# VincentStimper/normalizing-flows

Hardware: NVIDIA H100
Metric: samples/sec forward_kld, 32-layer RQ-NSF d=64 batch=65536 (higher is better)
Workload: dtype f32

## Files before the change

normalizing-flows_b200/csrc/nfb_common.cuh:

```cuda
#pragma once
#include <cuda_runtime.h>
#include <cuda_bf16.h>
#include <cuda_fp16.h>
#include <stdint.h>
#include <stdio.h>

#define NFB_OK 0
#define NFB_ERR_CUDA 1
#define NFB_ERR_ARG 2
#define NFB_ERR_UNSUPPORTED 3
#define NFB_ERR_STATE 4

void nfb_set_error(const char* fmt, ...);

#define NFB_CUDA(call)                                                                   \
    do {                                                                                 \
        cudaError_t e__ = (call);                                                        \
        if (e__ != cudaSuccess) {                                                        \
            nfb_set_error("%s:%d: %s -> %s", __FILE__, __LINE__, #call,                  \
                          cudaGetErrorString(e__));                                      \
            return NFB_ERR_CUDA;                                                         \
        }                                                                                \
    } while (0)

// ... 51 lines not shown
        "selp.u32 %0, 1, 0, p;\n\t}"
        : "=r"(ok)
        : "r"(bar), "r"(parity)
        : "memory");
    return ok != 0;
}
static __device__ __noinline__ void fail_timeout(int* err, int tag) {
    if (err) atomicExch(err, tag);
    __threadfence_system();
    asm volatile("trap;");
}

__device__ __forceinline__ void mbar_wait(uint32_t bar, uint32_t parity, int* err, int tag) {
    if (mbar_try_wait(bar, parity)) return;
    long long t0 = clock64();
    while (!mbar_try_wait(bar, parity)) {
        if (clock64() - t0 > 4000000000LL) fail_timeout(err, tag);
    }
}

__device__ __forceinline__ void mbar_wait_warp(uint32_t bar, uint32_t parity, int* err, int tag) {
    if ((threadIdx.x & 31) == 0 && !mbar_try_wait(bar, parity)) {
        long long t0 = clock64();
        while (!mbar_try_wait(bar, parity)) {
            if (clock64() - t0 > 4000000000LL) fail_timeout(err, tag);
        }
    }
    __syncwarp();
}

__device__ __forceinline__ void bulk_g2s(uint32_t dst_smem, const void* src, uint32_t bytes,
                                         uint32_t bar) {
    asm volatile(
        "cp.async.bulk.shared::cluster.global.mbarrier::complete_tx::bytes [%0], [%1], %2, [%3];"
        ::"r"(dst_smem), "l"(src), "r"(bytes), "r"(bar)
        : "memory");
}
__device__ __forceinline__ void fence_proxy_async_smem() {
    asm volatile("fence.proxy.async.shared::cta;" ::: "memory");
}

__device__ __forceinline__ uint64_t wgmma_desc(uint32_t smem_addr, uint32_t lbo16 = 1, uint32_t sbo16 = 64) {
    return (uint64_t)((smem_addr & 0x3FFFFu) >> 4) | ((uint64_t)lbo16 << 16) | ((uint64_t)sbo16 << 32) | (1ull << 62);
}
__device__ __forceinline__ void wgmma_fence() { asm volatile("wgmma.fence.sync.aligned;" ::: "memory"); }
__device__ __forceinline__ void wgmma_commit() { asm volatile("wgmma.commit_group.sync.aligned;" ::: "memory"); }
template <int N> __device__ __forceinline__ void wgmma_wait() {
    asm volatile("wgmma.wait_group.sync.aligned %0;" ::"n"(N) : "memory");
}
template <int R> __device__ __forceinline__ void wgmma_hold(float (&d)[R]) {
#pragma unroll
    for (int i = 0; i < R; ++i) asm volatile("" : "+f"(d[i])::"memory");
}
__device__ __forceinline__ void wgmma_f16_n64(float (&d)[32], uint64_t a, uint64_t b, uint32_t scale_d) {
    asm volatile(
        "{\n\t.reg .pred p;\n\tsetp.ne.b32 p, %34, 0;\n\t"
        "wgmma.mma_async.sync.aligned.m64n64k16.f32.f16.f16 "
        "{"
        "%0,%1,%2,%3,%4,%5,%6,%7,%8,%9,%10,%11,%12,%13,%14,%15,"
        "%16,%17,%18,%19,%20,%21,%22,%23,%24,%25,%26,%27,%28,%29,%30,%31"
        "}, %32, %33, p, 1, 1, 0, 0;\n\t}"
        : "+f"(d[0]), "+f"(d[1]), "+f"(d[2]), "+f"(d[3]), "+f"(d[4]), "+f"(d[5]), "+f"(d[6]), "+f"(d[7]), "+f"(d[8]),
          "+f"(d[9]), "+f"(d[10]), "+f"(d[11]), "+f"(d[12]), "+f"(d[13]), "+f"(d[14]), "+f"(d[15]), "+f"(d[16]),
          "+f"(d[17]), "+f"(d[18]), "+f"(d[19]), "+f"(d[20]), "+f"(d[21]), "+f"(d[22]), "+f"(d[23]), "+f"(d[24]),
          "+f"(d[25]), "+f"(d[26]), "+f"(d[27]), "+f"(d[28]), "+f"(d[29]), "+f"(d[30]), "+f"(d[31])
        : "l"(a), "l"(b), "r"(scale_d));
}
__device__ __forceinline__ void wgmma_f16_n96(float (&d)[48], uint64_t a, uint64_t b, uint32_t scale_d) {
    asm volatile(
        "{\n\t.reg .pred p;\n\tsetp.ne.b32 p, %50, 0;\n\t"
        "wgmma.mma_async.sync.aligned.m64n96k16.f32.f16.f16 "
        "{"
        "%0,%1,%2,%3,%4,%5,%6,%7,%8,%9,%10,%11,%12,%13,%14,%15,"
        "%16,%17,%18,%19,%20,%21,%22,%23,%24,%25,%26,%27,%28,%29,%30,%31,"
        "%32,%33,%34,%35,%36,%37,%38,%39,%40,%41,%42,%43,%44,%45,%46,%47"
        "}, %48, %49, p, 1, 1, 0, 0;\n\t}"
        : "+f"(d[0]), "+f"(d[1]), "+f"(d[2]), "+f"(d[3]), "+f"(d[4]), "+f"(d[5]), "+f"(d[6]), "+f"(d[7]), "+f"(d[8]),
          "+f"(d[9]), "+f"(d[10]), "+f"(d[11]), "+f"(d[12]), "+f"(d[13]), "+f"(d[14]), "+f"(d[15]), "+f"(d[16]),
          "+f"(d[17]), "+f"(d[18]), "+f"(d[19]), "+f"(d[20]), "+f"(d[21]), "+f"(d[22]), "+f"(d[23]), "+f"(d[24]),
          "+f"(d[25]), "+f"(d[26]), "+f"(d[27]), "+f"(d[28]), "+f"(d[29]), "+f"(d[30]), "+f"(d[31]), "+f"(d[32]),
          "+f"(d[33]), "+f"(d[34]), "+f"(d[35]), "+f"(d[36]), "+f"(d[37]), "+f"(d[38]), "+f"(d[39]), "+f"(d[40]),
          "+f"(d[41]), "+f"(d[42]), "+f"(d[43]), "+f"(d[44]), "+f"(d[45]), "+f"(d[46]), "+f"(d[47])
        : "l"(a), "l"(b), "r"(scale_d));
}
__device__ __forceinline__ void wgmma_f16_n96_zero(float (&d)[48], uint64_t a, uint64_t b) {
    asm volatile(
        "wgmma.mma_async.sync.aligned.m64n96k16.f32.f16.f16 "
        "{"
        "%0,%1,%2,%3,%4,%5,%6,%7,%8,%9,%10,%11,%12,%13,%14,%15,"
        "%16,%17,%18,%19,%20,%21,%22,%23,%24,%25,%26,%27,%28,%29,%30,%31,"
        "%32,%33,%34,%35,%36,%37,%38,%39,%40,%41,%42,%43,%44,%45,%46,%47"
        "}, %48, %49, 0, 1, 1, 0, 0;"
        : "=f"(d[0]), "=f"(d[1]), "=f"(d[2]), "=f"(d[3]), "=f"(d[4]), "=f"(d[5]), "=f"(d[6]), "=f"(d[7]), "=f"(d[8]),
          "=f"(d[9]), "=f"(d[10]), "=f"(d[11]), "=f"(d[12]), "=f"(d[13]), "=f"(d[14]), "=f"(d[15]), "=f"(d[16]),
          "=f"(d[17]), "=f"(d[18]), "=f"(d[19]), "=f"(d[20]), "=f"(d[21]), "=f"(d[22]), "=f"(d[23]), "=f"(d[24]),
          "=f"(d[25]), "=f"(d[26]), "=f"(d[27]), "=f"(d[28]), "=f"(d[29]), "=f"(d[30]), "=f"(d[31]), "=f"(d[32]),
          "=f"(d[33]), "=f"(d[34]), "=f"(d[35]), "=f"(d[36]), "=f"(d[37]), "=f"(d[38]), "=f"(d[39]), "=f"(d[40]),
          "=f"(d[41]), "=f"(d[42]), "=f"(d[43]), "=f"(d[44]), "=f"(d[45]), "=f"(d[46]), "=f"(d[47])
        : "l"(a), "l"(b));
}
template <int TA = 0, int TB = 0>
__device__ __forceinline__ void wgmma_bf16_n64(float (&d)[32], uint64_t a, uint64_t b, uint32_t scale_d, uint32_t on = 1) {
    asm volatile(
        "{\n\t.reg .pred p, q;\n\tsetp.ne.b32 p, %34, 0;\n\tsetp.ne.b32 q, %37, 0;\n\t"
        "@q wgmma.mma_async.sync.aligned.m64n64k16.f32.bf16.bf16 "
        "{"
        "%0,%1,%2,%3,%4,%5,%6,%7,%8,%9,%10,%11,%12,%13,%14,%15,"
        "%16,%17,%18,%19,%20,%21,%22,%23,%24,%25,%26,%27,%28,%29,%30,%31"
        "}, %32, %33, p, 1, 1, %35, %36;\n\t}"
        : "+f"(d[0]), "+f"(d[1]), "+f"(d[2]), "+f"(d[3]), "+f"(d[4]), "+f"(d[5]), "+f"(d[6]), "+f"(d[7]), "+f"(d[8]),
          "+f"(d[9]), "+f"(d[10]), "+f"(d[11]), "+f"(d[12]), "+f"(d[13]), "+f"(d[14]), "+f"(d[15]), "+f"(d[16]),
          "+f"(d[17]), "+f"(d[18]), "+f"(d[19]), "+f"(d[20]), "+f"(d[21]), "+f"(d[22]), "+f"(d[23]), "+f"(d[24]),
          "+f"(d[25]), "+f"(d[26]), "+f"(d[27]), "+f"(d[28]), "+f"(d[29]), "+f"(d[30]), "+f"(d[31])
        : "l"(a), "l"(b), "r"(scale_d), "n"(TA), "n"(TB), "r"(on));
}
template <int TA = 0, int TB = 0>
__device__ __forceinline__ void wgmma_bf16_n128(float (&d)[64], uint64_t a, uint64_t b, uint32_t scale_d, uint32_t on = 1) {
    asm volatile(
        "{\n\t.reg .pred p, q;\n\tsetp.ne.b32 p, %66, 0;\n\tsetp.ne.b32 q, %69, 0;\n\t"
        "@q wgmma.mma_async.sync.aligned.m64n128k16.f32.bf16.bf16 "
        "{"
        "%0,%1,%2,%3,%4,%5,%6,%7,%8,%9,%10,%11,%12,%13,%14,%15,"
        "%16,%17,%18,%19,%20,%21,%22,%23,%24,%25,%26,%27,%28,%29,%30,%31,"
        "%32,%33,%34,%35,%36,%37,%38,%39,%40,%41,%42,%43,%44,%45,%46,%47,"
        "%48,%49,%50,%51,%52,%53,%54,%55,%56,%57,%58,%59,%60,%61,%62,%63"
        "}, %64, %65, p, 1, 1, %67, %68;\n\t}"
        : "+f"(d[0]), "+f"(d[1]), "+f"(d[2]), "+f"(d[3]), "+f"(d[4]), "+f"(d[5]), "+f"(d[6]), "+f"(d[7]), "+f"(d[8]),
          "+f"(d[9]), "+f"(d[10]), "+f"(d[11]), "+f"(d[12]), "+f"(d[13]), "+f"(d[14]), "+f"(d[15]), "+f"(d[16]),
          "+f"(d[17]), "+f"(d[18]), "+f"(d[19]), "+f"(d[20]), "+f"(d[21]), "+f"(d[22]), "+f"(d[23]), "+f"(d[24]),
          "+f"(d[25]), "+f"(d[26]), "+f"(d[27]), "+f"(d[28]), "+f"(d[29]), "+f"(d[30]), "+f"(d[31]), "+f"(d[32]),
          "+f"(d[33]), "+f"(d[34]), "+f"(d[35]), "+f"(d[36]), "+f"(d[37]), "+f"(d[38]), "+f"(d[39]), "+f"(d[40]),
          "+f"(d[41]), "+f"(d[42]), "+f"(d[43]), "+f"(d[44]), "+f"(d[45]), "+f"(d[46]), "+f"(d[47]), "+f"(d[48]),
          "+f"(d[49]), "+f"(d[50]), "+f"(d[51]), "+f"(d[52]), "+f"(d[53]), "+f"(d[54]), "+f"(d[55]), "+f"(d[56]),
          "+f"(d[57]), "+f"(d[58]), "+f"(d[59]), "+f"(d[60]), "+f"(d[61]), "+f"(d[62]), "+f"(d[63])
        : "l"(a), "l"(b), "r"(scale_d), "n"(TA), "n"(TB), "r"(on));
}

template <int N> __device__ __forceinline__ void setmaxnreg_dec() {
    asm volatile("setmaxnreg.dec.sync.aligned.u32 %0;" ::"n"(N));
}
template <int N> __device__ __forceinline__ void setmaxnreg_inc() {
    asm volatile("setmaxnreg.inc.sync.aligned.u32 %0;" ::"n"(N));
}

__device__ __forceinline__ uint32_t pack_bf16x2(float lo_elem, float hi_elem) {
    uint32_t r;
    asm("cvt.rn.bf16x2.f32 %0, %1, %2;" : "=r"(r) : "f"(hi_elem), "f"(lo_elem));
    return r;
}
__device__ __forceinline__ uint32_t pack_f16x2(float lo_elem, float hi_elem) {
    uint32_t r;
    asm("cvt.rn.f16x2.f32 %0, %1, %2;" : "=r"(r) : "f"(hi_elem), "f"(lo_elem));
    return r;
}
__device__ __forceinline__ float2 unpack_f16x2(uint32_t h) {
    return __half22float2(*reinterpret_cast<const __half2*>(&h));
}

__device__ __forceinline__ float warp_sum(float v) {
#pragma unroll
    for (int o = 16; o > 0; o >>= 1) v += __shfl_xor_sync(0xffffffffu, v, o);
    return v;
}

}
```

normalizing-flows_b200/csrc/nfb_fused_rqs.cu:

```cuda
#include <type_traits>

#include "nfb_kernels.h"
#include "nfb_spline.cuh"

namespace nfb {

constexpr int kRows = kFusedTileRows;
constexpr int kCons = 256;
constexpr int kFusedThreads = kCons + 128;
constexpr int kProducerRegs = 24, kConsumerRegs = 240;
constexpr uint32_t kTileA = 8192;
constexpr uint32_t kSlotBytes = 32768;
constexpr uint32_t kSlots = 3;
constexpr uint32_t kOffW = 8 * kTileA;
constexpr uint32_t kOffX = kOffW + kSlots * kSlotBytes;
constexpr int kStgLd = 52;
constexpr uint32_t kStgBytes = kRows * kStgLd * 4;
constexpr uint32_t kOffStg = kOffX + kRows * 64 * 4;
constexpr uint32_t kOffMisc = kOffStg + 2 * kStgBytes;
constexpr uint32_t kOffBars = kOffMisc + 4 * kRows * 4;
constexpr uint32_t kNumBars = 10;
constexpr uint32_t kOffUnitQ = kOffBars + kNumBars * 8;
constexpr uint32_t kFusedSmem = kOffUnitQ + 32;
static_assert(kFusedSmem <= 232448, "shared memory budget");
static_assert(2 * kFusedFeaturesPerChunk * 24 * 64 * 4 <= (int)kSlotBytes, "final-layer record must fit a ring slot");

constexpr int kBarWFull = 0 , kBarWEmpty = 3 , kBarUnit = 6 ;

__device__ __forceinline__ uint32_t xs_index(int r, int c) { return r * 64 + (c ^ (r & 31)); }

__device__ __forceinline__ uint32_t a_chunk_off(int r, int c8) {
    return (r >> 3) * 1024 + (r & 7) * 128 + ((c8 ^ (r & 7)) << 4);
}

__device__ __forceinline__ void st_shared_v4(uint32_t addr, uint32_t a, uint32_t b, uint32_t c,
                                             uint32_t d) {
    asm volatile("st.shared.v4.b32 [%0], {%1,%2,%3,%4};" ::"r"(addr), "r"(a), "r"(b), "r"(c), "r"(d)
                 : "memory");
}
__device__ __forceinline__ void st_shared_b32(uint32_t addr, uint32_t v) {
    asm volatile("st.shared.b32 [%0], %1;" ::"r"(addr), "r"(v) : "memory");
}
__device__ __forceinline__ void cons_bar_sync() {
    asm volatile("bar.sync 1, %0;" ::"n"(kCons) : "memory");
}
constexpr int kBarStgFull = 2, kBarStgFree = 3;
template <int ID> __device__ __forceinline__ void stg_bar_arrive() {
    __threadfence_block();
    asm volatile("bar.arrive %0, %1;" ::"n"(ID), "n"(kCons) : "memory");
}
template <int ID> __device__ __forceinline__ void stg_bar_wait() {
    asm volatile("bar.sync %0, %1;" ::"n"(ID), "n"(kCons) : "memory");
}
__device__ __forceinline__ void mbar_arrive_if(uint32_t bar, bool pred) {
    asm volatile("{\n\t.reg .pred p;\n\tsetp.ne.b32 p, %1, 0;\n\t@p mbarrier.arrive.shared::cta.b64 _, [%0];\n\t}"
                 ::"r"(bar), "r"((uint32_t)pred) : "memory");
}

__device__ __forceinline__ void split_store8(const float* v, uint32_t t0, uint32_t t1, uint32_t off) {
    uint32_t h[4], l[4];
#pragma unroll
    for (int i = 0; i < 4; ++i) {
        const float a = v[2 * i], b = v[2 * i + 1];
        h[i] = pack_f16x2(a, b);
        const float2 hf = unpack_f16x2(h[i]);
        l[i] = pack_f16x2(a - hf.x, b - hf.y);
    }
    st_shared_v4(t0 + off, h[0], h[1], h[2], h[3]);
    st_shared_v4(t1 + off, l[0], l[1], l[2], l[3]);
}
template <typename T> __device__ __forceinline__ T uniform(T v) {
    return (T)__shfl_sync(0xffffffffu, (int)v, 0);
}
__device__ __forceinline__ float pow2i(int e) { return __uint_as_float((uint32_t)(127 + e) << 23); }

struct MmaOps { uint32_t a_hi, a_lo, w_hi, w_lo; bool first; uint32_t on, slabs; };
template <int SLABS, bool QUAD, int NREG, bool FIRST = false>
__device__ __forceinline__ void mma_record(float (&acc)[NREG], const MmaOps& x) {
    static_assert(NREG == 32 || NREG == 48, "N = 64 or 96");
    static_assert(!FIRST || NREG == 48, "an opening record of its own: the final layer's N = 96 products");
    const uint64_t ah = wgmma_desc(x.a_hi), al = wgmma_desc(x.a_lo), bh = wgmma_desc(x.w_hi), bl = wgmma_desc(x.w_lo);
    auto pass = [&](uint64_t a, uint64_t b, bool opens) {
#pragma unroll
        for (int s = 0; s < SLABS; ++s) {
            const uint32_t sd = opens && s == 0 && x.first ? 0u : 1u;
            if constexpr (NREG == 32) wgmma_f16_n64(acc, a + 2 * s, b + 2 * s, sd);
            else if (FIRST && opens && s == 0) wgmma_f16_n96_zero(acc, a, b);
            else wgmma_f16_n96(acc, a + 2 * s, b + 2 * s, FIRST ? 1u : sd);
        }
    };
    pass(ah, bh, true);
    pass(al, bh, false);
    pass(ah, bl, false);
    if constexpr (QUAD) pass(al, bl, false);
}

enum { kClkClaim,
       kClkLoad,
       kClkLu,
       kClkHidRing,
       kClkHidMma,
       kClkHidEpi,
       kClkFinRing,
       kClkFinMma,
       kClkFinTail,
       kClkFinStage,
       kClkFinSpline,
       kClkStore,
       kClkProdEmpty,
       kClkProdOther,
       kClkUnits,
       kClkCount };
template <int P> using ClkPhase = std::integral_constant<int, P>;
#ifdef NFB_PHASE_CLOCKS
__device__ unsigned long long g_phase_clocks[3][kClkCount];
struct PhaseClock {
    uint32_t last, sum[kClkCount];
    __device__ PhaseClock() {
        last = (uint32_t)clock64();
#pragma unroll
        for (int i = 0; i < kClkCount; ++i) sum[i] = 0;
    }
    template <int P> __device__ __forceinline__ void stamp() {
        const uint32_t t = (uint32_t)clock64();
        sum[P] += t - last;
        last = t;
    }
    __device__ void flush(int role) const {
#pragma unroll
        for (int i = 0; i < kClkCount; ++i) atomicAdd(&g_phase_clocks[role][i], (unsigned long long)sum[i]);
    }
};
#define NFB_CLK_BEGIN() PhaseClock clk
#define NFB_CLK(P) clk.template stamp<P>()
#define NFB_CLK_UNIT() (++clk.sum[kClkUnits])
#define NFB_CLK_END(role, pred) do { if (pred) clk.flush(role); } while (0)
#else
#define NFB_CLK_BEGIN() ((void)0)
#define NFB_CLK(P) ((void)0)
#define NFB_CLK_UNIT() ((void)0)
#define NFB_CLK_END(role, pred) ((void)0)
#endif

template <bool SAMPLE>
__global__ void __launch_bounds__(kFusedThreads, 1) fused_rqs_kernel(const FusedParams p) {
    extern __shared__ __align__(1024) uint8_t smem[];
    const uint32_t sbase = smem_u32(smem);
    const int warp = uniform((int)(threadIdx.x >> 5)), lane = threadIdx.x & 31;
    float* xs = reinterpret_cast<float*>(smem + kOffX);
    float* ldsum = reinterpret_cast<float*>(smem + kOffMisc);
    int* rowexp = reinterpret_cast<int*>(smem + kOffMisc + 3 * kRows * 4);
    float* rowmax = reinterpret_cast<float*>(smem + kOffStg);
    const uint32_t bars = sbase + kOffBars;
    auto bar = [bars](int i) { return bars + 8u * i; };

    if ((sbase & 1023u) != 0) {
        if (threadIdx.x == 0 && p.err) atomicExch(p.err, 900);
        return;
    }
    if (threadIdx.x == 0) {
        for (int i = 0; i < (int)kSlots; ++i) {
            mbar_init(bar(kBarWFull + i), 1);
            mbar_init(bar(kBarWEmpty + i), 2);
        }
        for (int i = 0; i < 4; ++i) mbar_init(bar(kBarUnit + i), 1);
        fence_mbar_init();
    }
    __syncthreads();

    volatile int* unit_q = reinterpret_cast<volatile int*>(smem + kOffUnitQ);
    if (warp >= kCons / 32) {
        setmaxnreg_dec<kProducerRegs>();
        if (warp != kCons / 32) return;
        const long long n_tiles = (p.rows + kRows - 1) / kRows;
        const long long n_units = n_tiles * p.n_layers;
        auto decode = [&](long long u, int& cursor, int& layer, long long& tile) {
            if (!p.wave_order) {
                layer = (int)(u / n_tiles);
                tile = u - (long long)layer * n_tiles;
                return;
            }
            while (cursor + 1 < p.wave_elems && u >= (long long)__ldg(p.wave_order + 2 * (cursor + 1) + 1)) ++cursor;
            const uint32_t w = __ldg(p.wave_order + 2 * cursor);
            layer = (int)(w & 0xffu);
            tile = (long long)(w >> 8) * p.wave_tpg + (u - (long long)__ldg(p.wave_order + 2 * cursor + 1));
        };
        uint32_t slot = 0, par = 0;
        int wcur = 0;
        NFB_CLK_BEGIN();
        for (uint32_t ui = 0;; ++ui) {
            long long u;
            if (p.ticket) {
                int t = 0;
                if (lane == 0) t = atomicAdd(p.ticket, 1);
                u = (long long)__shfl_sync(0xffffffffu, t, 0);
            } else {
                u = (long long)blockIdx.x + (long long)ui * gridDim.x;
            }
            const bool more = u < n_units;
            int ulayer = -1;
            long long utile = 0;
            if (more) decode(u, wcur, ulayer, utile);
            if (lane == 0) {
                unit_q[2 * (ui & 3u)] = ulayer;
                unit_q[2 * (ui & 3u) + 1] = (int)utile;
                mbar_arrive(bar(kBarUnit + (ui & 3u)));
            }
            __syncwarp();
            if (!more) break;
            NFB_CLK_UNIT();
            const FusedLayer& L = p.layers[ulayer];
            const FusedStep* steps = L.steps;
            const int n_steps = L.n_steps;
            const int lu_steps = L.has_lu ? 1 : 0;
            const int reps = (SAMPLE && L.ar_passes > 0) ? L.ar_passes : 1;
            const int total = n_steps ? lu_steps + reps * (n_steps - lu_steps) : 0;
            const uint32_t lu_bytes = L.has_lu ? 2u * 8192u : 0u;
            int s = 0;
            uint32_t off = 0;
            uint32_t bytes = total ? (uint32_t)__ldg(&steps[0].bytes16) << 4 : 0u;
            for (int i = 0; i < total; ++i) {
                int sn = s + 1;
                uint32_t offn = off + bytes;
                if (sn == n_steps) { sn = lu_steps; offn = lu_bytes; }
                const uint32_t nbytes = i + 1 < total ? (uint32_t)__ldg(&steps[sn].bytes16) << 4 : 0u;
                NFB_CLK(kClkProdOther);
                mbar_wait(bar(kBarWEmpty + slot), par ^ 1, p.err, 100 + slot);
                NFB_CLK(kClkProdEmpty);
                if (elect_one_sync()) {
                    mbar_expect_tx(bar(kBarWFull + slot), bytes);
                    bulk_g2s(sbase + kOffW + slot * kSlotBytes, L.wstream + off, bytes, bar(kBarWFull + slot));
                }
                __syncwarp();
                s = sn;
                off = offn;
                bytes = nbytes;
                if (++slot == kSlots) { slot = 0; par ^= 1; }
            }
        }
        NFB_CLK(kClkProdOther);
        NFB_CLK_END(2, lane == 0);
        return;
    }

    setmaxnreg_inc<kConsumerRegs>();
    const int et = threadIdx.x;
    const int wg = uniform(et >> 7);
    const int wl = warp & 3;
    const int ra = 16 * wl + (lane >> 2);
    const int rb = ra + 8;
    const int cq = 2 * (lane & 3);
    const uint32_t aA = sbase;
    float* stg0 = reinterpret_cast<float*>(smem + kOffStg);
    uint32_t slot = 0, wpar = 0;
    NFB_CLK_BEGIN();

    for (uint32_t ui = 0;; ++ui) {
        mbar_wait(bar(kBarUnit + (ui & 3u)), (ui >> 2) & 1u, p.err, 600 + (int)(ui & 3u));
        const int layer = uniform(unit_q[2 * (ui & 3u)]);
        const long long tile = uniform(unit_q[2 * (ui & 3u) + 1]);
        if (layer < 0) break;
        NFB_CLK_UNIT();
        const FusedLayer& L = p.layers[layer];
        const int D = L.D;
        auto own = [&](int q) { return uniform((int)L.own[wg][q]); };
        const int n_steps = uniform(L.n_steps), lu_steps = uniform(L.has_lu ? 1 : 0);
        const int n_hidden = uniform(L.n_hidden), n_pairs = uniform(L.n_chunks >> 1);
        int sidx = 0;
        auto hand_back = [&](auto arrivals, int s, bool pred) {
#pragma unroll
            for (int i = 0; i < decltype(arrivals)::value; ++i) mbar_arrive_if(bar(kBarWEmpty + s), pred && (et & 127) == 0);
        };
        auto walk_records = [&](auto issue, auto arrivals, auto clk_ring, auto clk_mma, int& prev, auto open,
                                auto retire) {
            auto record = [&](auto first) {
                union { uint2 raw; FusedStep s; } st;
                st.raw = __ldg(reinterpret_cast<const uint2*>(L.steps) + sidx);
                st.raw.x = uniform(st.raw.x);
                st.raw.y = uniform(st.raw.y);
                sidx = sidx + 1 == n_steps ? lu_steps : sidx + 1;
                NFB_CLK(decltype(clk_mma)::value);
                mbar_wait(bar(kBarWFull + slot), wpar, p.err, 220 + slot);
                NFB_CLK(decltype(clk_ring)::value);
                wgmma_fence();
                const bool last = issue(st.s, first);
                if constexpr (decltype(first)::value) NFB_CLK(decltype(clk_mma)::value);
                wgmma_wait<1>();
                hand_back(arrivals, prev < 0 ? 0 : prev, prev >= 0);
                if constexpr (decltype(first)::value) NFB_CLK(kClkFinTail);
                prev = (int)slot;
                if (++slot == kSlots) { slot = 0; wpar ^= 1; }
                return last;
            };
            bool last = false;
            if constexpr (decltype(open)::value) {
                last = record(std::true_type());
                retire();
            }
            while (!last) last = record(std::false_type());
        };
        auto run_records = [&](auto issue, auto arrivals, auto clk_ring, auto clk_mma) {
            int prev = -1;
            walk_records(issue, arrivals, clk_ring, clk_mma, prev, std::false_type(), [] {});
            wgmma_wait<0>();
            hand_back(arrivals, prev, true);
            NFB_CLK(decltype(clk_mma)::value);
        };
        auto half_ops = [&](const FusedStep& s, int h, bool live) {
            const uint32_t kc = h ? s.kc1 : s.kc, fl = h ? s.flags1 : s.flags;
            const uint32_t w = sbase + kOffW + slot * kSlotBytes + ((fl & kStepHalf) ? 0u : (uint32_t)h * s.n8 * 1024u);
            return MmaOps{aA + kc * kTileA, aA + (4 + kc) * kTileA, w, w + ((uint32_t)s.bytes16 << 3), (fl & kStepFirst) != 0,
                          (uint32_t)(live && !(fl & kStepSkip)), 4u - ((fl >> kStepSlabShift) & 3u)};
        };
        auto run_slice = [&](auto& acc, bool live, auto quad, auto clk_ring, auto clk_mma) {
            run_records([&](const FusedStep& s, auto) {
                const MmaOps x = half_ops(s, wg, live);
                if (x.on) mma_record<4, decltype(quad)::value>(acc, x);
                wgmma_commit();
                return ((wg ? s.flags1 : s.flags) & kStepLast) != 0;
            }, std::integral_constant<int, 1>(), clk_ring, clk_mma);
            wgmma_hold(acc);
        };
        using NoQuad = std::integral_constant<bool, false>;

        float* zdst = p.zout + (long long)layer * p.z_stride;
        const float* zsrc = layer == 0 ? p.zin : p.zout + (long long)(layer - 1) * p.z_stride;
        const long long row0 = tile * kRows;
        const int r = et & (kRows - 1);
        const int rq = et >> 6;
        const long long grow = row0 + r;
        const bool row_live = grow < p.rows;

        if (layer > 0) {
            if (lane == 0) {
                const int* flag = p.progress + tile;
                int seen;
                const long long t0 = clock64();
                do {
                    asm volatile("ld.acquire.gpu.global.s32 %0, [%1];" : "=r"(seen) : "l"(flag) : "memory");
                    if (seen < layer && clock64() - t0 > 4000000000LL) fail_timeout(p.err, 500);
                } while (seen < layer);
            }
            __syncwarp();
            {
                int seen;
                asm volatile("ld.acquire.gpu.global.s32 %0, [%1];" : "=r"(seen) : "l"(p.progress + tile) : "memory");
                if (seen < layer) fail_timeout(p.err, 501);
            }
        }
        if (layer == 0 && p.in_ready) {
            const int need = (int)min(row0 + kRows, p.rows);
            if (lane == 0) {
                int seen;
                const long long t0 = clock64();
                do {
                    asm volatile("ld.acquire.sys.global.s32 %0, [%1];" : "=r"(seen) : "l"(p.in_ready) : "memory");
                    if (seen < need && clock64() - t0 > 20000000000LL) fail_timeout(p.err, 510);
                } while (seen < need);
            }
            __syncwarp();
            {
                int seen;
                asm volatile("ld.acquire.sys.global.s32 %0, [%1];" : "=r"(seen) : "l"(p.in_ready) : "memory");
                if (seen < need) fail_timeout(p.err, 511);
            }
        }
        NFB_CLK(kClkClaim);
        float lq_old = 0.f;
        if (rq == 2 && row_live && (layer > 0 || p.accumulate)) lq_old = __ldcg(p.logq + grow);
        if (D == 64) {
            float4 v[kRows * 16 / kCons];
#pragma unroll
            for (int k = 0; k < kRows * 16 / kCons; ++k) {
                const int i4 = et + k * kCons, rr = i4 >> 4;
                const long long gr = row0 + rr;
                v[k] = gr < p.rows ? __ldcg(reinterpret_cast<const float4*>(zsrc + gr * 64) + (i4 & 15))
                                   : make_float4(0.f, 0.f, 0.f, 0.f);
            }
#pragma unroll
            for (int k = 0; k < kRows * 16 / kCons; ++k) {
                const int i4 = et + k * kCons, rr = i4 >> 4, c0 = (i4 & 15) * 4;
                xs[xs_index(rr, c0)] = v[k].x;
                xs[xs_index(rr, c0 + 1)] = v[k].y;
                xs[xs_index(rr, c0 + 2)] = v[k].z;
                xs[xs_index(rr, c0 + 3)] = v[k].w;
                float m = fmaxf(fmaxf(fabsf(v[k].x), fabsf(v[k].y)), fmaxf(fabsf(v[k].z), fabsf(v[k].w)));
                m = fmaxf(m, __shfl_xor_sync(0xffffffffu, m, 1));
                m = fmaxf(m, __shfl_xor_sync(0xffffffffu, m, 2));
                m = fmaxf(m, __shfl_xor_sync(0xffffffffu, m, 4));
                m = fmaxf(m, __shfl_xor_sync(0xffffffffu, m, 8));
                if ((et & 15) == 0) rowmax[rr] = m;
            }
        } else {
            for (int i = et; i < kRows * D; i += kCons) {
                const int rr = i / D, cc = i - rr * D;
                const long long gr = row0 + rr;
                xs[xs_index(rr, cc)] = gr < p.rows ? __ldcg(zsrc + gr * D + cc) : 0.f;
            }
        }
        cons_bar_sync();
        auto set_row_exp = [&](float zmax) {
            int e = (int)((__float_as_uint(zmax) >> 23) & 0xffu) - 126;
            rowexp[r] = max(0, min(126, e));
        };
        if (rq == 0) {
            float zmax = 0.f;
            if (D == 64) zmax = rowmax[r];
            else
                for (int c = 0; c < D; ++c) zmax = fmaxf(zmax, fabsf(xs[xs_index(r, c)]));
            set_row_exp(zmax);
        }
        cons_bar_sync();
        auto ru = [&](float s, int row) { return s * pow2i(-rowexp[row]); };
        auto ruinv = [&](float s, int row) { return s * pow2i(rowexp[row]); };
        auto get_x = [&](int c) -> float { return xs[xs_index(r, c)]; };
        auto put_y = [&](int c, float y) { xs[xs_index(r, c)] = y; };
        const int ar = et >> 2, aq = et & 3;
        auto store_a = [&](auto value, float sc_base) {
            const float sc = ru(sc_base, ar);
            float v[16];
#pragma unroll
            for (int j = 0; j < 16; ++j) v[j] = value(aq * 16 + j) * sc;
#pragma unroll
            for (int g = 0; g < 2; ++g) split_store8(v + 8 * g, aA, aA + 4 * kTileA, a_chunk_off(ar, 2 * aq + g));
            fence_proxy_async_smem();
            cons_bar_sync();
        };
        auto build_a_net = [&]() {
            store_a([&](int k) {
                const int c = L.in_idx[k];
                return c >= 0 ? xs[xs_index(ar, c)] : 0.f;
            }, L.a_sc[1]);
        };
        float ladsum = 0.f, lad_even = 0.f;
        const bool folded = uniform(!SAMPLE && L.has_lu && L.fold_lu);
        if (lu_steps) {
            store_a([&](int k) { return k < D ? xs[xs_index(ar, k)] : 0.f; }, L.a_sc[0]);
            float acc[32];
            NFB_CLK(kClkLoad);
            run_slice(acc, wg == 0, std::integral_constant<bool, true>(), ClkPhase<kClkLu>(), ClkPhase<kClkLu>());
            if (wg == 0) {
                const float ia = ruinv(L.a_inv[0], ra), ib = ruinv(L.a_inv[0], rb);
#pragma unroll
                for (int i = 0; i < 32; ++i) {
                    const int c = 8 * (i >> 2) + cq + (i & 1);
                    const int rr = (i & 2) ? rb : ra;
                    if (c < D) xs[xs_index(rr, c)] = fmaf(acc[i], (i & 2) ? ib : ia, __ldg(L.bias_lu + c));
                }
            }
            cons_bar_sync();
            NFB_CLK(kClkLu);
        }
        auto store_tile = [&]() {
            if (D == 64) {
#pragma unroll
                for (int k = 0; k < kRows * 16 / kCons; ++k) {
                    const int i4 = et + k * kCons, rr = i4 >> 4, c0 = (i4 & 15) * 4;
                    const long long gr = row0 + rr;
                    const float4 v = make_float4(xs[xs_index(rr, c0)], xs[xs_index(rr, c0 + 1)],
                                                 xs[xs_index(rr, c0 + 2)], xs[xs_index(rr, c0 + 3)]);
                    if (gr < p.rows) __stcg(reinterpret_cast<float4*>(zdst + gr * 64) + (i4 & 15), v);
                }
            } else {
                for (int i = et; i < kRows * D; i += kCons) {
                    const int rr = i / D, cc = i - rr * D;
                    const long long gr = row0 + rr;
                    if (gr < p.rows) __stcg(zdst + gr * D + cc, xs[xs_index(rr, cc)]);
                }
            }
        };
        const bool arsamp = uniform(SAMPLE && L.ar_passes > 0);
        const int reps = uniform(arsamp ? L.ar_passes : 1);
        if (arsamp) {
            store_tile();
            if (rq == 0) {
                float zmax = L.tail;
                for (int c = 0; c < D; ++c) zmax = fmaxf(zmax, fabsf(xs[xs_index(r, c)]));
                set_row_exp(zmax);
            }
            cons_bar_sync();
            for (int i = et; i < kRows * 64; i += kCons) xs[i] = 0.f;
            cons_bar_sync();
        }
        for (int rep = 0; rep < reps; ++rep) {
            if (rep > 0) {
                ladsum = 0.f;
                cons_bar_sync();
            }
            auto uncond = [&]() {
                for (int i = rq; i < L.n_id; i += kCons / kRows) {
                    const int c = L.id_idx[i];
                    const float* tb = L.uncond + i * 23;
                    auto acc = [tb](int k) { return __ldg(tb + k); };
                    float y, l;
                    rqs_eval<8, SAMPLE>(get_x(c), acc, L.tail, 1.0f, y, l);
                    put_y(c, y);
                    ladsum += l;
                }
            };
            if (SAMPLE && L.n_id > 0) {
                uncond();
                cons_bar_sync();
            }
            if (!folded) build_a_net();
            if (!SAMPLE && L.n_id > 0) uncond();
            NFB_CLK(kClkLoad);

            if (wg == 0) ldsum[rq * kRows + r] = ladsum;
            float hres[2][32] = {};
            for (int ph = 0; ph < n_hidden; ++ph) {
                const bool t_phase = (ph & 1) != 0;
                const bool relu = ph + 1 < n_hidden;
                float tacc[2][32] = {};
#pragma unroll
                for (int q = 0; q < 2; ++q) {
                    const int j = own(q);
                    if (q == 0 || j >= 0) {
                        if (t_phase) run_slice(tacc[q], j >= 0, NoQuad(), ClkPhase<kClkHidRing>(), ClkPhase<kClkHidMma>());
                        else run_slice(hres[q], j >= 0, NoQuad(), ClkPhase<kClkHidRing>(), ClkPhase<kClkHidMma>());
                    }
                }
                cons_bar_sync();
                const float inv_a = ruinv(L.a_inv[1 + ph], ra), inv_b = ruinv(L.a_inv[1 + ph], rb);
                const float sc_a = ru(L.a_sc[2 + ph], ra), sc_b = ru(L.a_sc[2 + ph], rb);
                auto epilogue = [&](const float (&acc)[32], int j) {
                    const float* bias = L.bias_h + ph * 256 + 64 * j;
#pragma unroll
                    for (int g = 0; g < 8; ++g) {
                        const float2 b2 = __ldg(reinterpret_cast<const float2*>(bias + 8 * g + cq));
#pragma unroll
                        for (int hb = 0; hb < 2; ++hb) {
                            const int rr = hb ? rb : ra;
                            float v0 = fmaf(acc[4 * g + 2 * hb], hb ? inv_b : inv_a, b2.x);
                            float v1 = fmaf(acc[4 * g + 2 * hb + 1], hb ? inv_b : inv_a, b2.y);
                            if (relu) { v0 = fmaxf(v0, 0.f); v1 = fmaxf(v1, 0.f); }
                            v0 *= hb ? sc_b : sc_a;
                            v1 *= hb ? sc_b : sc_a;
                            const uint32_t hi = pack_f16x2(v0, v1);
                            const float2 hf = unpack_f16x2(hi);
                            const uint32_t off = (rr >> 3) * 1024 + (rr & 7) * 128 + ((g ^ (rr & 7)) << 4) + cq * 2;
                            st_shared_b32(aA + j * kTileA + off, hi);
                            st_shared_b32(aA + (4 + j) * kTileA + off, pack_f16x2(v0 - hf.x, v1 - hf.y));
                        }
                    }
                };
#pragma unroll
                for (int q = 0; q < 2; ++q) {
                    const int j = own(q);
                    if (j >= 0) {
                        if (t_phase) epilogue(tacc[q], j);
                        else epilogue(hres[q], j);
                    }
                }
                fence_proxy_async_smem();
                cons_bar_sync();
                NFB_CLK(kClkHidEpi);
            }

            if (wg == 0) {
                static_assert(kFusedFeaturesPerChunk == 2, "a final-layer record is one N = 96 product");
                auto products = [&](float (&acc)[48]) {
                    return [&](const FusedStep& s, auto first) {
                        constexpr bool F = decltype(first)::value;
                        const MmaOps x = half_ops(s, 0, true), x1 = half_ops(s, 1, true);
                        const uint32_t n = max(x.on ? x.slabs : 0u, x1.on ? x1.slabs : 0u);
                        switch (n) {
                            case 1: mma_record<1, false, 48, F>(acc, x); wgmma_commit(); break;
                            case 2: mma_record<2, false, 48, F>(acc, x); wgmma_commit(); break;
                            case 3: mma_record<3, false, 48, F>(acc, x); wgmma_commit(); break;
                            default: mma_record<4, false, 48, F>(acc, x); wgmma_commit(); break;
                        }
                        return (s.flags & kStepLast) != 0;
                    };
                };
                const float fin_a = ruinv(L.a_inv[1 + n_hidden], ra), fin_b = ruinv(L.a_inv[1 + n_hidden], rb);
                float2 fbias[2][6];
                auto load_bias = [&](int ci) {
                    if (ci >= n_pairs) return;
#pragma unroll
                    for (int h = 0; h < 2; ++h)
#pragma unroll
                        for (int g = 0; g < 6; ++g)
                            fbias[h][g] = __ldg(reinterpret_cast<const float2*>(L.bias_f + (2 * ci + h) * L.F * 24 + 8 * g + cq));
                };
                auto stage = [&](float (&acc)[48], int ci) {
                    wgmma_hold(acc);
                    if (ci > 0) stg_bar_wait<kBarStgFree>();
#pragma unroll
                    for (int i = 0; i < 24; i += 2) {
                        const int g = i >> 2;
                        const float u = (i & 2) ? fin_b : fin_a;
                        float* dst = stg0 + ((i & 2) ? rb : ra) * kStgLd + 8 * g + cq;
                        *reinterpret_cast<float2*>(dst) =
                            make_float2(fmaf(acc[i], u, fbias[0][g].x), fmaf(acc[i + 1], u, fbias[0][g].y));
                        *reinterpret_cast<float2*>(dst + kRows * kStgLd) =
                            make_float2(fmaf(acc[24 + i], u, fbias[1][g].x), fmaf(acc[25 + i], u, fbias[1][g].y));
                    }
                    stg_bar_arrive<kBarStgFull>();
                    load_bias(ci + 1);
                    NFB_CLK(kClkFinStage);
                };
                using Two = std::integral_constant<int, 2>;
                int prev = -1;
                auto pair = [&](float (&acc)[48], float (&done)[48], int ci) {
                    walk_records(products(acc), Two(), ClkPhase<kClkFinRing>(), ClkPhase<kClkFinMma>(), prev,
                                 std::true_type(), [&] { stage(done, ci - 1); });
                };
                auto finish = [&](float (&acc)[48], int ci) {
                    wgmma_wait<0>();
                    hand_back(Two(), prev, true);
                    NFB_CLK(kClkFinTail);
                    stage(acc, ci);
                };
                float accA[48], accB[48];
                if (n_pairs > 0) {
                    load_bias(0);
                    walk_records(products(accA), Two(), ClkPhase<kClkFinRing>(), ClkPhase<kClkFinMma>(), prev,
                                 std::true_type(), [] {});
                    for (int ci = 1;; ci += 2) {
                        if (ci == n_pairs) { finish(accA, ci - 1); break; }
                        pair(accB, accA, ci);
                        if (ci + 1 == n_pairs) { finish(accB, ci); break; }
                        pair(accA, accB, ci + 1);
                    }
                }
            } else {
                if (n_pairs > 0) {
                    const uint32_t adv = slot + (uint32_t)(n_steps - sidx);
                    slot = adv % kSlots;
                    wpar ^= (adv / kSlots) & 1u;
                    sidx = lu_steps;
                }
                const int f = (et >> 6) & 1;
                lad_even = ldsum[f * kRows + r];
                const int F = L.F, T = L.T;
                for (int ci = 0; ci < n_pairs; ++ci) {
                    stg_bar_wait<kBarStgFull>();
                    float pv[2][24];
#pragma unroll
                    for (int h = 0; h < 2; ++h) {
                        const float4* sp = reinterpret_cast<const float4*>(stg0 + (h * kRows + r) * kStgLd + 24 * f);
#pragma unroll
                        for (int q = 0; q < 6; ++q) {
                            const float4 s4 = sp[q];
                            pv[h][4 * q] = s4.x;
                            pv[h][4 * q + 1] = s4.y;
                            pv[h][4 * q + 2] = s4.z;
                            pv[h][4 * q + 3] = s4.w;
                        }
                    }
                    if (ci + 1 < n_pairs) stg_bar_arrive<kBarStgFree>();
                    NFB_CLK(kClkFinStage);
                    const int t0 = 2 * ci * F + f;
                    auto splines = [&](auto lanes) {
                        constexpr int N = decltype(lanes)::value;
                        int col[N];
                        float xin[N], y[N], l[N];
#pragma unroll
                        for (int h = 0; h < N; ++h) {
                            col[h] = L.tr_idx[t0 + h * F];
                            xin[h] = get_x(col[h]);
                            if (arsamp) xin[h] = row_live ? __ldcg(zdst + grow * D + col[h]) : 0.f;
                        }
                        rqs_core_lanes<N, 8, SAMPLE>(xin, [&pv](int h, int i) { return pv[h][i]; },
                                                     [&pv](int h, int i) { return pv[h][8 + i]; },
                                                     [&pv](int h, int i) { return pv[h][16 + i]; }, L.tail, y, l);
#pragma unroll
                        for (int h = 0; h < N; ++h) put_y(col[h], y[h]);
                        lad_even += l[0];
                        if constexpr (N == 2) ladsum += l[1];
                    };
                    if (t0 + F < T) splines(std::integral_constant<int, 2>());
                    else if (t0 < T) splines(std::integral_constant<int, 1>());
                    NFB_CLK(kClkFinSpline);
                }
            }
            cons_bar_sync();
        }
        NFB_CLK(kClkFinStage);
        if (rq == 3) {
            ldsum[r] = lad_even;
            ldsum[kRows + r] = ladsum;
        }
        cons_bar_sync();
        if (rq == 2 && row_live) {
            const float tot = lad_even + ldsum[r] + ladsum + ldsum[kRows + r] +
                              (L.lu_logdet ? __ldg(L.lu_logdet) : 0.f);
            __stcg(p.logq + grow, tot + lq_old);
        }
        store_tile();
        if (p.progress) __threadfence();
        cons_bar_sync();
        if (p.progress && et == 0) {
            __threadfence();
            asm volatile("st.release.gpu.global.s32 [%0], %1;" ::"l"(p.progress + tile), "r"(layer + 1) : "memory");
        }
        NFB_CLK(kClkStore);
    }
    NFB_CLK_END(wg, (et & 127) == 0);
}

// ... 173 lines not shown
```

Before: 5.360 million.

## Overlap hidden-layer epilogue with second GEMM and store activations via stmatrix

Restructures the hidden-layer loop so the two output slices a warpgroup owns are computed back to back, with the first slice's epilogue (bias, ReLU, f16 hi/lo split) running while the second slice's wgmma is in flight. Packed results are held in registers and written to the swizzled A tiles with stmatrix instead of scalar shared stores. The epilogue is templated on how many slices a warpgroup owns, and the first product uses a zero-init wgmma rather than a runtime scale flag. It trades more live registers and code size for less serialization between MMA and epilogue and fewer shared-store instructions.

```diff
diff --git a/normalizing-flows_b200/csrc/nfb_common.cuh b/normalizing-flows_b200/csrc/nfb_common.cuh
--- a/normalizing-flows_b200/csrc/nfb_common.cuh
+++ b/normalizing-flows_b200/csrc/nfb_common.cuh
@@ -157,6 +157,19 @@
           "+f"(d[33]), "+f"(d[34]), "+f"(d[35]), "+f"(d[36]), "+f"(d[37]), "+f"(d[38]), "+f"(d[39]), "+f"(d[40]),
           "+f"(d[41]), "+f"(d[42]), "+f"(d[43]), "+f"(d[44]), "+f"(d[45]), "+f"(d[46]), "+f"(d[47])
         : "l"(a), "l"(b), "r"(scale_d));
+}
+__device__ __forceinline__ void wgmma_f16_n64_zero(float (&d)[32], uint64_t a, uint64_t b) {
+    asm volatile(
+        "wgmma.mma_async.sync.aligned.m64n64k16.f32.f16.f16 "
+        "{"
+        "%0,%1,%2,%3,%4,%5,%6,%7,%8,%9,%10,%11,%12,%13,%14,%15,"
+        "%16,%17,%18,%19,%20,%21,%22,%23,%24,%25,%26,%27,%28,%29,%30,%31"
+        "}, %32, %33, 0, 1, 1, 0, 0;"
+        : "=f"(d[0]), "=f"(d[1]), "=f"(d[2]), "=f"(d[3]), "=f"(d[4]), "=f"(d[5]), "=f"(d[6]), "=f"(d[7]), "=f"(d[8]),
+          "=f"(d[9]), "=f"(d[10]), "=f"(d[11]), "=f"(d[12]), "=f"(d[13]), "=f"(d[14]), "=f"(d[15]), "=f"(d[16]),
+          "=f"(d[17]), "=f"(d[18]), "=f"(d[19]), "=f"(d[20]), "=f"(d[21]), "=f"(d[22]), "=f"(d[23]), "=f"(d[24]),
+          "=f"(d[25]), "=f"(d[26]), "=f"(d[27]), "=f"(d[28]), "=f"(d[29]), "=f"(d[30]), "=f"(d[31])
+        : "l"(a), "l"(b));
 }
 __device__ __forceinline__ void wgmma_f16_n96_zero(float (&d)[48], uint64_t a, uint64_t b) {
     asm volatile(
@@ -231,6 +244,10 @@
 __device__ __forceinline__ float2 unpack_f16x2(uint32_t h) {
     return __half22float2(*reinterpret_cast<const __half2*>(&h));
 }
+__device__ __forceinline__ void stmatrix_x4(uint32_t addr, uint32_t r0, uint32_t r1, uint32_t r2, uint32_t r3) {
+    asm volatile("stmatrix.sync.aligned.m8n8.x4.shared.b16 [%0], {%1, %2, %3, %4};" ::"r"(addr), "r"(r0), "r"(r1),
+                 "r"(r2), "r"(r3) : "memory");
+}
 
 __device__ __forceinline__ float warp_sum(float v) {
 #pragma unroll
diff --git a/normalizing-flows_b200/csrc/nfb_fused_rqs.cu b/normalizing-flows_b200/csrc/nfb_fused_rqs.cu
--- a/normalizing-flows_b200/csrc/nfb_fused_rqs.cu
+++ b/normalizing-flows_b200/csrc/nfb_fused_rqs.cu
@@ -38,9 +38,6 @@
     asm volatile("st.shared.v4.b32 [%0], {%1,%2,%3,%4};" ::"r"(addr), "r"(a), "r"(b), "r"(c), "r"(d)
                  : "memory");
 }
-__device__ __forceinline__ void st_shared_b32(uint32_t addr, uint32_t v) {
-    asm volatile("st.shared.b32 [%0], %1;" ::"r"(addr), "r"(v) : "memory");
-}
 __device__ __forceinline__ void cons_bar_sync() {
     asm volatile("bar.sync 1, %0;" ::"n"(kCons) : "memory");
 }
@@ -74,19 +71,21 @@
 }
 __device__ __forceinline__ float pow2i(int e) { return __uint_as_float((uint32_t)(127 + e) << 23); }
 
-struct MmaOps { uint32_t a_hi, a_lo, w_hi, w_lo; bool first; uint32_t on, slabs; };
+struct MmaOps { uint32_t a_hi, a_lo, w_hi, w_lo, on, slabs; };
 template <int SLABS, bool QUAD, int NREG, bool FIRST = false>
 __device__ __forceinline__ void mma_record(float (&acc)[NREG], const MmaOps& x) {
     static_assert(NREG == 32 || NREG == 48, "N = 64 or 96");
-    static_assert(!FIRST || NREG == 48, "an opening record of its own: the final layer's N = 96 products");
     const uint64_t ah = wgmma_desc(x.a_hi), al = wgmma_desc(x.a_lo), bh = wgmma_desc(x.w_hi), bl = wgmma_desc(x.w_lo);
     auto pass = [&](uint64_t a, uint64_t b, bool opens) {
 #pragma unroll
         for (int s = 0; s < SLABS; ++s) {
-            const uint32_t sd = opens && s == 0 && x.first ? 0u : 1u;
-            if constexpr (NREG == 32) wgmma_f16_n64(acc, a + 2 * s, b + 2 * s, sd);
-            else if (FIRST && opens && s == 0) wgmma_f16_n96_zero(acc, a, b);
-            else wgmma_f16_n96(acc, a + 2 * s, b + 2 * s, FIRST ? 1u : sd);
+            if constexpr (NREG == 32) {
+                if (FIRST && opens && s == 0) wgmma_f16_n64_zero(acc, a, b);
+                else wgmma_f16_n64(acc, a + 2 * s, b + 2 * s, 1u);
+            } else {
+                if (FIRST && opens && s == 0) wgmma_f16_n96_zero(acc, a, b);
+                else wgmma_f16_n96(acc, a + 2 * s, b + 2 * s, 1u);
+            }
         }
     };
     pass(ah, bh, true);
@@ -111,7 +110,10 @@
        kClkProdOther,
        kClkUnits,
        kClkCount };
-template <int P> using ClkPhase = std::integral_constant<int, P>;
+template <int RING, int MMA, int TAIL> struct WalkClk { static constexpr int ring = RING, mma = MMA, tail = TAIL; };
+using LuClk = WalkClk<kClkLu, kClkLu, kClkLu>;
+using HidClk = WalkClk<kClkHidRing, kClkHidMma, kClkHidMma>;
+using FinClk = WalkClk<kClkFinRing, kClkFinMma, kClkFinTail>;
 #ifdef NFB_PHASE_CLOCKS
 __device__ unsigned long long g_phase_clocks[3][kClkCount];
 struct PhaseClock {
@@ -271,23 +273,23 @@
 #pragma unroll
             for (int i = 0; i < decltype(arrivals)::value; ++i) mbar_arrive_if(bar(kBarWEmpty + s), pred && (et & 127) == 0);
         };
-        auto walk_records = [&](auto issue, auto arrivals, auto clk_ring, auto clk_mma, int& prev, auto open,
-                                auto retire) {
+        auto walk_records = [&](auto issue, auto arrivals, auto phases, int& prev, auto open, auto retire) {
+            using Clk = decltype(phases);
             auto record = [&](auto first) {
                 union { uint2 raw; FusedStep s; } st;
                 st.raw = __ldg(reinterpret_cast<const uint2*>(L.steps) + sidx);
                 st.raw.x = uniform(st.raw.x);
                 st.raw.y = uniform(st.raw.y);
                 sidx = sidx + 1 == n_steps ? lu_steps : sidx + 1;
-                NFB_CLK(decltype(clk_mma)::value);
+                NFB_CLK(Clk::mma);
                 mbar_wait(bar(kBarWFull + slot), wpar, p.err, 220 + slot);
-                NFB_CLK(decltype(clk_ring)::value);
+                NFB_CLK(Clk::ring);
                 wgmma_fence();
                 const bool last = issue(st.s, first);
-                if constexpr (decltype(first)::value) NFB_CLK(decltype(clk_mma)::value);
+                if constexpr (decltype(first)::value) NFB_CLK(Clk::mma);
                 wgmma_wait<1>();
                 hand_back(arrivals, prev < 0 ? 0 : prev, prev >= 0);
-                if constexpr (decltype(first)::value) NFB_CLK(kClkFinTail);
+                if constexpr (decltype(first)::value) NFB_CLK(Clk::tail);
                 prev = (int)slot;
                 if (++slot == kSlots) { slot = 0; wpar ^= 1; }
                 return last;
@@ -299,28 +301,33 @@
             }
             while (!last) last = record(std::false_type());
         };
-        auto run_records = [&](auto issue, auto arrivals, auto clk_ring, auto clk_mma) {
-            int prev = -1;
-            walk_records(issue, arrivals, clk_ring, clk_mma, prev, std::false_type(), [] {});
-            wgmma_wait<0>();
-            hand_back(arrivals, prev, true);
-            NFB_CLK(decltype(clk_mma)::value);
-        };
-        auto half_ops = [&](const FusedStep& s, int h, bool live) {
+        auto half_ops = [&](const FusedStep& s, int h) {
             const uint32_t kc = h ? s.kc1 : s.kc, fl = h ? s.flags1 : s.flags;
             const uint32_t w = sbase + kOffW + slot * kSlotBytes + ((fl & kStepHalf) ? 0u : (uint32_t)h * s.n8 * 1024u);
-            return MmaOps{aA + kc * kTileA, aA + (4 + kc) * kTileA, w, w + ((uint32_t)s.bytes16 << 3), (fl & kStepFirst) != 0,
-                          (uint32_t)(live && !(fl & kStepSkip)), 4u - ((fl >> kStepSlabShift) & 3u)};
+            return MmaOps{aA + kc * kTileA, aA + (4 + kc) * kTileA, w, w + ((uint32_t)s.bytes16 << 3),
+                          (uint32_t)!(fl & kStepSkip), 4u - ((fl >> kStepSlabShift) & 3u)};
         };
-        auto run_slice = [&](auto& acc, bool live, auto quad, auto clk_ring, auto clk_mma) {
-            run_records([&](const FusedStep& s, auto) {
-                const MmaOps x = half_ops(s, wg, live);
-                if (x.on) mma_record<4, decltype(quad)::value>(acc, x);
-                wgmma_commit();
+        auto slice_products = [&](float (&acc)[32], auto opens, auto quad) {
+            return [&](const FusedStep& s, auto first) {
+                constexpr bool Q = decltype(quad)::value;
+                const MmaOps x = half_ops(s, wg);
+                if constexpr (decltype(first)::value && decltype(opens)::value) {
+                    mma_record<4, Q, 32, true>(acc, x);
+                    wgmma_commit();
+                } else if (x.on) {
+                    mma_record<4, Q, 32>(acc, x);
+                    wgmma_commit();
+                } else {
+                    wgmma_commit();
+                }
                 return ((wg ? s.flags1 : s.flags) & kStepLast) != 0;
-            }, std::integral_constant<int, 1>(), clk_ring, clk_mma);
-            wgmma_hold(acc);
+            };
         };
+        auto no_products = [&](const FusedStep& s, auto) {
+            wgmma_commit();
+            return ((wg ? s.flags1 : s.flags) & kStepLast) != 0;
+        };
+        using One = std::integral_constant<int, 1>;
         using NoQuad = std::integral_constant<bool, false>;
 
         float* zdst = p.zout + (long long)layer * p.z_stride;
@@ -436,10 +443,15 @@
         const bool folded = uniform(!SAMPLE && L.has_lu && L.fold_lu);
         if (lu_steps) {
             store_a([&](int k) { return k < D ? xs[xs_index(ar, k)] : 0.f; }, L.a_sc[0]);
-            float acc[32];
             NFB_CLK(kClkLoad);
-            run_slice(acc, wg == 0, std::integral_constant<bool, true>(), ClkPhase<kClkLu>(), ClkPhase<kClkLu>());
+            int prev = -1;
             if (wg == 0) {
+                float acc[32];
+                walk_records(slice_products(acc, std::true_type(), std::true_type()), One(), LuClk(), prev,
+                             std::true_type(), [] {});
+                wgmma_wait<0>();
+                hand_back(One(), prev, true);
+                wgmma_hold(acc);
                 const float ia = ruinv(L.a_inv[0], ra), ib = ruinv(L.a_inv[0], rb);
 #pragma unroll
                 for (int i = 0; i < 32; ++i) {
@@ -447,6 +459,10 @@
                     const int rr = (i & 2) ? rb : ra;
                     if (c < D) xs[xs_index(rr, c)] = fmaf(acc[i], (i & 2) ? ib : ia, __ldg(L.bias_lu + c));
                 }
+            } else {
+                walk_records(no_products, One(), LuClk(), prev, std::false_type(), [] {});
+                wgmma_wait<0>();
+                hand_back(One(), prev, true);
             }
             cons_bar_sync();
             NFB_CLK(kClkLu);
@@ -507,62 +523,81 @@
             NFB_CLK(kClkLoad);
 
             if (wg == 0) ldsum[rq * kRows + r] = ladsum;
-            float hres[2][32] = {};
-            for (int ph = 0; ph < n_hidden; ++ph) {
-                const bool t_phase = (ph & 1) != 0;
-                const bool relu = ph + 1 < n_hidden;
-                float tacc[2][32] = {};
-#pragma unroll
-                for (int q = 0; q < 2; ++q) {
-                    const int j = own(q);
-                    if (q == 0 || j >= 0) {
-                        if (t_phase) run_slice(tacc[q], j >= 0, NoQuad(), ClkPhase<kClkHidRing>(), ClkPhase<kClkHidMma>());
-                        else run_slice(hres[q], j >= 0, NoQuad(), ClkPhase<kClkHidRing>(), ClkPhase<kClkHidMma>());
-                    }
-                }
-                cons_bar_sync();
-                const float inv_a = ruinv(L.a_inv[1 + ph], ra), inv_b = ruinv(L.a_inv[1 + ph], rb);
-                const float sc_a = ru(L.a_sc[2 + ph], ra), sc_b = ru(L.a_sc[2 + ph], rb);
-                auto epilogue = [&](const float (&acc)[32], int j) {
-                    const float* bias = L.bias_h + ph * 256 + 64 * j;
-#pragma unroll
-                    for (int g = 0; g < 8; ++g) {
-                        const float2 b2 = __ldg(reinterpret_cast<const float2*>(bias + 8 * g + cq));
-#pragma unroll
-                        for (int hb = 0; hb < 2; ++hb) {
-                            const int rr = hb ? rb : ra;
-                            float v0 = fmaf(acc[4 * g + 2 * hb], hb ? inv_b : inv_a, b2.x);
-                            float v1 = fmaf(acc[4 * g + 2 * hb + 1], hb ? inv_b : inv_a, b2.y);
+            auto hidden = [&](auto ns) {
+                constexpr int NA = decltype(ns)::value > 0 ? decltype(ns)::value : 1;
+                auto gemm = [&](auto& acc, auto opens, int ph) {
+                    constexpr int NS = decltype(ns)::value, NA = NS > 0 ? NS : 1;
+                    const bool relu = ph + 1 < n_hidden;
+                    const float inv_a = ruinv(L.a_inv[1 + ph], ra), inv_b = ruinv(L.a_inv[1 + ph], rb);
+                    const float sc_a = ru(L.a_sc[2 + ph], ra), sc_b = ru(L.a_sc[2 + ph], rb);
+                    float2 bias[NA][8];
+#pragma unroll
+                    for (int q = 0; q < NS; ++q)
+#pragma unroll
+                        for (int g = 0; g < 8; ++g)
+                            bias[q][g] = __ldg(reinterpret_cast<const float2*>(L.bias_h + ph * 256 + 64 * own(q) + 8 * g + cq));
+                    uint32_t pk[NA][2][16];
+                    auto pack = [&](int q, float (&a)[32]) {
+                        wgmma_hold(a);
+#pragma unroll
+                        for (int p = 0; p < 16; ++p) {
+                            const int g = p >> 1, hb = p & 1;
+                            float v0 = fmaf(a[2 * p], hb ? inv_b : inv_a, bias[q][g].x);
+                            float v1 = fmaf(a[2 * p + 1], hb ? inv_b : inv_a, bias[q][g].y);
                             if (relu) { v0 = fmaxf(v0, 0.f); v1 = fmaxf(v1, 0.f); }
                             v0 *= hb ? sc_b : sc_a;
                             v1 *= hb ? sc_b : sc_a;
                             const uint32_t hi = pack_f16x2(v0, v1);
                             const float2 hf = unpack_f16x2(hi);
-                            const uint32_t off = (rr >> 3) * 1024 + (rr & 7) * 128 + ((g ^ (rr & 7)) << 4) + cq * 2;
-                            st_shared_b32(aA + j * kTileA + off, hi);
-                            st_shared_b32(aA + (4 + j) * kTileA + off, pack_f16x2(v0 - hf.x, v1 - hf.y));
+                            pk[q][0][p] = hi;
+                            pk[q][1][p] = pack_f16x2(v0 - hf.x, v1 - hf.y);
                         }
+                    };
+                    int prev = -1;
+                    if constexpr (NS == 0) {
+                        walk_records(no_products, One(), HidClk(), prev, std::false_type(), [] {});
+                    } else {
+                        walk_records(slice_products(acc[0], opens, NoQuad()), One(), HidClk(), prev, std::true_type(),
+                                     [] {});
+                        if constexpr (NS == 2)
+                            walk_records(slice_products(acc[1], opens, NoQuad()), One(), HidClk(), prev, std::true_type(),
+                                         [&] { pack(0, acc[0]); NFB_CLK(kClkHidEpi); });
                     }
+                    wgmma_wait<0>();
+                    hand_back(One(), prev, true);
+                    NFB_CLK(kClkHidMma);
+                    if constexpr (NS > 0) pack(NS - 1, acc[NS - 1]);
+                    cons_bar_sync();
+#pragma unroll
+                    for (int q = 0; q < NS; ++q)
+#pragma unroll
+                        for (int h = 0; h < 2; ++h)
+#pragma unroll
+                            for (int k = 0; k < 4; ++k)
+                                stmatrix_x4(aA + (4 * h + own(q)) * kTileA + a_chunk_off(16 * wl + (lane & 15), 2 * k + (lane >> 4)),
+                                            pk[q][h][4 * k], pk[q][h][4 * k + 1], pk[q][h][4 * k + 2], pk[q][h][4 * k + 3]);
+                    fence_proxy_async_smem();
+                    cons_bar_sync();
+                    NFB_CLK(kClkHidEpi);
                 };
-#pragma unroll
-                for (int q = 0; q < 2; ++q) {
-                    const int j = own(q);
-                    if (j >= 0) {
-                        if (t_phase) epilogue(tacc[q], j);
-                        else epilogue(hres[q], j);
-                    }
+                float hres[NA][32];
+                gemm(hres, std::true_type(), 0);
+                for (int ph = 1; ph + 1 < n_hidden; ph += 2) {
+                    float tacc[NA][32];
+                    gemm(tacc, std::true_type(), ph);
+                    gemm(hres, std::false_type(), ph + 1);
                 }
-                fence_proxy_async_smem();
-                cons_bar_sync();
-                NFB_CLK(kClkHidEpi);
-            }
+            };
+            if (own(0) < 0) hidden(std::integral_constant<int, 0>());
+            else if (own(1) < 0) hidden(std::integral_constant<int, 1>());
+            else hidden(std::integral_constant<int, 2>());
 
             if (wg == 0) {
                 static_assert(kFusedFeaturesPerChunk == 2, "a final-layer record is one N = 96 product");
                 auto products = [&](float (&acc)[48]) {
                     return [&](const FusedStep& s, auto first) {
                         constexpr bool F = decltype(first)::value;
-                        const MmaOps x = half_ops(s, 0, true), x1 = half_ops(s, 1, true);
+                        const MmaOps x = half_ops(s, 0), x1 = half_ops(s, 1);
                         const uint32_t n = max(x.on ? x.slabs : 0u, x1.on ? x1.slabs : 0u);
                         switch (n) {
                             case 1: mma_record<1, false, 48, F>(acc, x); wgmma_commit(); break;
@@ -602,9 +637,8 @@
                 };
                 using Two = std::integral_constant<int, 2>;
                 int prev = -1;
-                auto pair = [&](float (&acc)[48], float (&done)[48], int ci) {
-                    walk_records(products(acc), Two(), ClkPhase<kClkFinRing>(), ClkPhase<kClkFinMma>(), prev,
-                                 std::true_type(), [&] { stage(done, ci - 1); });
+                auto pair = [&](float (&acc)[48], float (&done)[48], int ci) __attribute__((always_inline)) {
+                    walk_records(products(acc), Two(), FinClk(), prev, std::true_type(), [&] { stage(done, ci - 1); });
                 };
                 auto finish = [&](float (&acc)[48], int ci) {
                     wgmma_wait<0>();
@@ -615,8 +649,7 @@
                 float accA[48], accB[48];
                 if (n_pairs > 0) {
                     load_bias(0);
-                    walk_records(products(accA), Two(), ClkPhase<kClkFinRing>(), ClkPhase<kClkFinMma>(), prev,
-                                 std::true_type(), [] {});
+                    walk_records(products(accA), Two(), FinClk(), prev, std::true_type(), [] {});
                     for (int ci = 1;; ci += 2) {
                         if (ci == n_pairs) { finish(accA, ci - 1); break; }
                         pair(accB, accA, ci);
```

Measured after the change: 5.527 million (median of 6 runs). 3.1% higher.
